# FutureSDR/FutureSDR

Hardware: AMD Instinct MI355X
Metric: MSample/s through 127-tap C32 FIR→decim4→1k-FFT flowgraph @1/2/4/8 GPU (higher is better)
Workload: dtype f32; 1 GPU; fir127_decim4_fft1024; taps1=127, taps2=127, decim=4, fft_len=1024, parallelism=1 independent channels

## Files before the change

### futuresdr_amd/csrc/futuresdr_hip.hip

```cpp
#include <hip/hip_runtime.h>

#include <atomic>
#include <condition_variable>
#include <cstdio>
#include <cstring>
#include <cstdlib>
#include <deque>
#include <mutex>
#include <vector>
#include <algorithm>
#include <cmath>

#include "../../include/futuresdr_hip.h"


static thread_local char g_err[512];
static thread_local const char* g_err_ptr = "";

static void set_err(const char* msg) {
    snprintf(g_err, sizeof(g_err), "%s", msg);
    g_err_ptr = g_err;
}

extern "C" const char* fsdr_last_error(void) { return g_err_ptr; }
// ... 1667 lines not shown
    return ((((unsigned)(DFIRT_TILE + tpd + 12)) + 31u) & ~31u) + 8u;
}

template <int TPD>
__global__ __launch_bounds__(DFIRT_BLOCK) void k_fir_decim4_tpl(
    const float2* __restrict__ in, float2* __restrict__ out,
    const float* __restrict__ rtv ,
    long long n_out, long long n_in_valid) {
    static_assert(TPD % 4 == 0, "TPD must be a multiple of 4");
    const unsigned SP = dfirt_sp(TPD);
    extern __shared__ __attribute__((aligned(16))) char smem[];
    float* planes = (float*)smem;
    float* s_rt = planes + 4u * SP;

    const int tid = threadIdx.x;
    const unsigned span = 3 + 4 * (DFIRT_TILE + TPD + 8);
    for (long long tile = blockIdx.x;
         tile * (long long)DFIRT_TILE < n_out; tile += gridDim.x) {
        const long long out_base = tile * DFIRT_TILE;
        const long long in_base = out_base * 4;
        const unsigned eb = (unsigned)tid * DFIRT_R;
        float2 a01r = make_float2(0.f, 0.f), a23r = a01r;
        float2 a01i = a01r, a23i = a01r;
#pragma unroll
        for (int half = 0; half < 2; half++) {
            for (unsigned idx = tid; 2 * idx + 3 < span;
                 idx += DFIRT_BLOCK) {
                unsigned i = idx >> 1, vloc = idx & 1u;
                unsigned rel = 3 + 4 * i + 2 * half + vloc;
                if (rel >= span) continue;
                long long g = in_base + rel;
                float2 x = (g < n_in_valid) ? in[g] : make_float2(0.f, 0.f);
                planes[vloc * SP + i] = x.x;
                planes[(2 + vloc) * SP + i] = x.y;
            }
            if (half == 0)
                for (int i = tid; i < 4 * (TPD + 4); i += DFIRT_BLOCK)
                    s_rt[i] = rtv[i];
            __syncthreads();
#pragma unroll
            for (int vloc = 0; vloc < 2; vloc++) {
                const float* pre = planes + (unsigned)vloc * SP;
                const float* pim = planes + (unsigned)(2 + vloc) * SP;
                const float* rt =
                    s_rt + (unsigned)(2 * half + vloc) * (TPD + 4);
                float4 r0 = *(const float4*)&pre[eb];
                float4 r1 = *(const float4*)&pre[eb + 4];
                float4 i0 = *(const float4*)&pim[eb];
                float4 i1 = *(const float4*)&pim[eb + 4];
                float4 hc = *(const float4*)&rt[0];
                constexpr int NG = TPD / 4;
#pragma unroll 4
                for (int m = 0; m < NG; m++) {
                    const float4 rn = *(const float4*)&pre[eb + 4 * m + 8];
                    const float4 in_ = *(const float4*)&pim[eb + 4 * m + 8];
                    const float4 h4 = *(const float4*)&rt[4 * m + 4];
                    const float wr[8] = {r0.x, r0.y, r0.z, r0.w,
                                         r1.x, r1.y, r1.z, r1.w};
                    const float wi[8] = {i0.x, i0.y, i0.z, i0.w,
                                         i1.x, i1.y, i1.z, i1.w};
                    const float ht[4] = {hc.x, hc.y, hc.z, hc.w};
#pragma unroll
                    for (int tl = 0; tl < 4; tl++) {
                        const float h = ht[tl];
                        a01r.x = fmaf(wr[tl], h, a01r.x);
                        a01r.y = fmaf(wr[tl + 1], h, a01r.y);
                        a23r.x = fmaf(wr[tl + 2], h, a23r.x);
                        a23r.y = fmaf(wr[tl + 3], h, a23r.y);
                        a01i.x = fmaf(wi[tl], h, a01i.x);
                        a01i.y = fmaf(wi[tl + 1], h, a01i.y);
                        a23i.x = fmaf(wi[tl + 2], h, a23i.x);
                        a23i.y = fmaf(wi[tl + 3], h, a23i.y);
                    }
                    r0 = r1; r1 = rn;
                    i0 = i1; i1 = in_;
                    hc = h4;
                }
            }
            __syncthreads();
        }
        const float ar[4] = {a01r.x, a01r.y, a23r.x, a23r.y};
        const float ai[4] = {a01i.x, a01i.y, a23i.x, a23i.y};
#pragma unroll
        for (int j = 0; j < DFIRT_R; j++) {
            long long o = out_base + eb + j;
            if (o < n_out) out[o] = make_float2(ar[j], ai[j]);
        }
    }
}

typedef void (*dfir_tpl_fn)(const float2*, float2*, const float*, long long,
                            long long);

__global__ void k_fir_decim_generic_cf32(const float2* __restrict__ in,
                                         float2* __restrict__ out,
                                         const float* __restrict__ taps,
                                         int n_taps, long long decim,
                                         long long n_out,
                                         long long n_in_valid) {
    long long stride = (long long)gridDim.x * blockDim.x;
    for (long long k = blockIdx.x * (long long)blockDim.x + threadIdx.x;
         k < n_out; k += stride) {
        float sre = 0.f, sim = 0.f;
        long long base = decim - 1 + k * decim;
        for (int t = 0; t < n_taps; t++) {
            float2 x = (base + t < n_in_valid) ? in[base + t]
                                               : make_float2(0.f, 0.f);
            float h = taps[n_taps - 1 - t];
            sre = fmaf(x.x, h, sre);
            sim = fmaf(x.y, h, sim);
        }
        out[k] = make_float2(sre, sim);
    }
}

__global__ __launch_bounds__(256) void k_fir_ccf32(
    const float2* __restrict__ in, float2* __restrict__ out,
    const float2* __restrict__ taps, int n_taps, long long n_out,
    long long n_in_valid) {
    const unsigned TILE = 1024;
    const unsigned elems = TILE + n_taps - 1;
    extern __shared__ __attribute__((aligned(16))) char smem[];
    float2* s_x = (float2*)smem;
    float2* s_h = s_x + elems;
    const int tid = threadIdx.x;
    for (long long tile = blockIdx.x; tile * (long long)TILE < n_out;
         tile += gridDim.x) {
        const long long out_base = tile * TILE;
        for (unsigned i = tid; i < elems; i += 256) {
            long long g = out_base + i;
            s_x[i] = (g < n_in_valid) ? in[g] : make_float2(0.f, 0.f);
        }
        for (int i = tid; i < n_taps; i += 256)
            s_h[i] = taps[n_taps - 1 - i];
        __syncthreads();
        for (int j = 0; j < 4; j++) {
            unsigned k = tid + j * 256;
            float sre = 0.f, sim = 0.f;
            for (int t = 0; t < n_taps; t++) {
                float2 x = s_x[k + t];
                float2 h = s_h[t];
                sre = fmaf(x.x, h.x, sre);
                sre = fmaf(-x.y, h.y, sre);
                sim = fmaf(x.x, h.y, sim);
                sim = fmaf(x.y, h.x, sim);
            }
            long long o = out_base + k;
            if (o < n_out) out[o] = make_float2(sre, sim);
        }
        __syncthreads();
    }
}

__global__ void k_moving_avg_chunks(const float* __restrict__ in,
                                    float* __restrict__ partial, int width,
                                    long long frames, int n_chunks,
                                    int chunk_frames, float decay) {
    if ((width & 3) == 0) {
        int w4 = width >> 2;
        long long id = blockIdx.x * (long long)blockDim.x + threadIdx.x;
        long long total = (long long)n_chunks * w4;
        long long stride = (long long)gridDim.x * blockDim.x;
        for (; id < total; id += stride) {
            int c = (int)(id / w4);
            int b4 = (int)(id - (long long)c * w4);
            long long f0 = (long long)c * chunk_frames;
            long long f1 = f0 + chunk_frames;
            if (f1 > frames) f1 = frames;
            float4 p = make_float4(0.f, 0.f, 0.f, 0.f);
            const float om = 1.0f - decay;
            for (long long f = f0; f < f1; f++) {
                float4 t = *(const float4*)&in[f * width + 4 * b4];
                p.x = isfinite(t.x) ? om * p.x + decay * t.x : om * p.x;
                p.y = isfinite(t.y) ? om * p.y + decay * t.y : om * p.y;
                p.z = isfinite(t.z) ? om * p.z + decay * t.z : om * p.z;
                p.w = isfinite(t.w) ? om * p.w + decay * t.w : om * p.w;
            }
            *(float4*)&partial[(long long)c * width + 4 * b4] = p;
        }
        return;
    }
    long long id = blockIdx.x * (long long)blockDim.x + threadIdx.x;
    long long total = (long long)n_chunks * width;
    long long stride = (long long)gridDim.x * blockDim.x;
    for (; id < total; id += stride) {
        int c = (int)(id / width);
        int b = (int)(id - (long long)c * width);
        long long f0 = (long long)c * chunk_frames;
        long long f1 = f0 + chunk_frames;
        if (f1 > frames) f1 = frames;
        float p = 0.f;
        for (long long f = f0; f < f1; f++) {
            float t = in[f * width + b];
            if (isfinite(t))
                p = (1.0f - decay) * p + decay * t;
            else
                p *= 1.0f - decay;
        }
        partial[(long long)c * width + b] = p;
    }
}

__global__ void k_moving_avg_combine(const float* __restrict__ partial,
                                     float* __restrict__ avg,
                                     float* __restrict__ out ,
                                     int width, long long frames,
                                     int n_chunks, int chunk_frames,
                                     float decay) {
    __shared__ float red[256];
    const int b = blockIdx.x;
    if (b >= width) return;
    const float om = 1.0f - decay;
    float acc = 0.f;
    for (int c = threadIdx.x; c < n_chunks; c += blockDim.x) {
        long long end = (long long)(c + 1) * chunk_frames;
        if (end > frames) end = frames;
        acc += powf(om, (float)(frames - end)) *
               partial[(long long)c * width + b];
    }
    red[threadIdx.x] = acc;
    __syncthreads();
    for (int s = 128; s > 0; s >>= 1) {
        if (threadIdx.x < s) red[threadIdx.x] += red[threadIdx.x + s];
        __syncthreads();
    }
    if (threadIdx.x == 0) {
        float a = powf(om, (float)frames) * avg[b] + red[0];
        avg[b] = a;
        if (out) out[b] = a;
    }
}

__global__ __launch_bounds__(256) void k_xlating_decim_ccf32(
    const float2* __restrict__ in, float2* __restrict__ out,
    const float2* __restrict__ taps , int n_taps,
    long long decim, long long n_out, long long n_in_valid, double theta,
    float p0r, float p0i) {
    extern __shared__ __attribute__((aligned(16))) char smem[];
    float2* s_h = (float2*)smem;
    for (int i = threadIdx.x; i < n_taps; i += blockDim.x) s_h[i] = taps[i];
    __syncthreads();
    long long stride = (long long)gridDim.x * blockDim.x;
    for (long long k = blockIdx.x * (long long)blockDim.x + threadIdx.x;
         k < n_out; k += stride) {
        float sre = 0.f, sim = 0.f;
        long long base = decim - 1 + k * decim;
        for (int t = 0; t < n_taps; t++) {
            float2 x = (base + t < n_in_valid) ? in[base + t]
                                               : make_float2(0.f, 0.f);
            float2 hh = s_h[t];
            sre = fmaf(x.x, hh.x, sre);
            sre = fmaf(-x.y, hh.y, sre);
            sim = fmaf(x.x, hh.y, sim);
            sim = fmaf(x.y, hh.x, sim);
        }
        double a = theta * (double)(k + 1);
        a -= 6.283185307179586 * floor(a * 0.15915494309189535);
        float s, cth;
        __sincosf((float)a, &s, &cth);
        float pr = cth * p0r - s * p0i;
        float pi = cth * p0i + s * p0r;
        out[k] = make_float2(sre * pr - sim * pi, sre * pi + sim * pr);
    }
}

#define XT_BLOCK 256
#define XT_R 2
#define XT_TILE (XT_BLOCK * XT_R)

__global__ __launch_bounds__(XT_BLOCK) void k_xlating_decim_tiled_ccf32(
    const float2* __restrict__ in, float2* __restrict__ out,
    const float2* __restrict__ taps , int n_taps,
    int decim, long long n_out, long long n_in_valid, double theta,
    float p0r, float p0i, int span) {
    extern __shared__ __attribute__((aligned(16))) char smem[];
    float* s_re = (float*)smem;
    float* s_im = s_re + plane_floats((unsigned)span);
    float* s_hr = s_im + plane_floats((unsigned)span);
    float* s_hi = s_hr + n_taps;
    for (int i = threadIdx.x; i < n_taps; i += XT_BLOCK) {
        s_hr[i] = taps[i].x;
        s_hi[i] = taps[i].y;
    }
    const long long tiles = (n_out + XT_TILE - 1) / XT_TILE;
    for (long long tile = blockIdx.x; tile < tiles; tile += gridDim.x) {
        const long long out_base = tile * XT_TILE;
        const long long in_base = decim - 1 + out_base * decim;
        __syncthreads();
        for (int i = threadIdx.x; i < span; i += XT_BLOCK) {
            long long g = in_base + i;
            float2 v = (g < n_in_valid) ? in[g] : make_float2(0.f, 0.f);
            s_re[lds_pad((unsigned)i)] = v.x;
            s_im[lds_pad((unsigned)i)] = v.y;
        }
        __syncthreads();
#pragma unroll
        for (int r = 0; r < XT_R; r++) {
            long long k = out_base + threadIdx.x + r * XT_BLOCK;
            if (k >= n_out) break;
            unsigned rel = (unsigned)((k - out_base) * decim);
            float sre = 0.f, sim = 0.f;
#pragma unroll 4
            for (int t = 0; t < n_taps; t++) {
                unsigned a = lds_pad(rel + (unsigned)t);
                float xr = s_re[a], xi = s_im[a];
                float hr = s_hr[t], hi = s_hi[t];
                sre = fmaf(xr, hr, sre);
                sre = fmaf(-xi, hi, sre);
                sim = fmaf(xr, hi, sim);
                sim = fmaf(xi, hr, sim);
            }
            double a = theta * (double)(k + 1);
            a -= 6.283185307179586 * floor(a * 0.15915494309189535);
            float s, cth;
            __sincosf((float)a, &s, &cth);
            float pr = cth * p0r - s * p0i;
            float pi = cth * p0i + s * p0r;
            out[k] = make_float2(sre * pr - sim * pi, sre * pi + sim * pr);
        }
    }
}

__global__ void k_cmul_conj(const float2* __restrict__ a,
                            const float2* __restrict__ b,
                            float2* __restrict__ o, long long n) {
    long long stride = (long long)gridDim.x * blockDim.x;
    for (long long i = blockIdx.x * (long long)blockDim.x + threadIdx.x;
         i < n; i += stride) {
        float2 x = a[i], y = b[i];
        o[i] = make_float2(x.x * y.x + x.y * y.y, x.y * y.x - x.x * y.y);
    }
}

__global__ void k_divide_mag(const float2* __restrict__ a,
                             const float* __restrict__ b,
                             float* __restrict__ o, long long n) {
    long long stride = (long long)gridDim.x * blockDim.x;
    for (long long i = blockIdx.x * (long long)blockDim.x + threadIdx.x;
         i < n; i += stride) {
        float2 x = a[i];
        o[i] = sqrtf(x.x * x.x + x.y * x.y) / b[i];
    }
}

__global__ void k_moving_sum(const float* __restrict__ in,
                             float* __restrict__ out, int width, int len,
                             long long n_out_items) {
    long long stride = (long long)gridDim.x * blockDim.x;
    long long total = n_out_items * width;
    for (long long id = blockIdx.x * (long long)blockDim.x + threadIdx.x;
         id < total; id += stride) {
        long long i = id / width;
        int q = (int)(id - i * width);
        float sum = 0.f;
        for (int t = 0; t < len; t++) sum += in[(i + t) * width + q];
        out[id] = sum;
    }
}

__global__ void k_pfb_dots(const float2* __restrict__ in,
                           float2* __restrict__ fb,
                           const float* __restrict__ part ,
                           int N, int tpf, int D, long long steps,
                           long long p_before, long long bufbase) {
    long long id = blockIdx.x * (long long)blockDim.x + threadIdx.x;
    long long total = steps * N;
    long long stride = (long long)gridDim.x * blockDim.x;
// ... 848 lines not shown

extern "C" fsdr_filter* fsdr_mag2_create(void) {
    fsdr_filter* f = create_common(K_MAG2);
    if (!f) return nullptr;
    f->item_out = 4;
    return f;
}

extern "C" fsdr_filter* fsdr_xlating_fir_cf32_create(const float* taps,
                                                     size_t n_taps,
                                                     size_t decimation,
                                                     float offset,
                                                     float sample_rate) {
    if (!taps || n_taps == 0 || decimation < 2) {
        set_err("xlating fir: taps required, decimation must be >= 2");
        return nullptr;
    }
    fsdr_filter* f = create_common(K_XLATING);
    if (!f) return nullptr;
    f->n_taps = n_taps;
    f->decim = decimation;
    std::vector<float2> bpf(n_taps);
    for (size_t i = 0; i < n_taps; i++) {
        float ang = (float)i * 6.2831853071795864769f * offset / sample_rate;
        float2 rot = make_float2(cosf(ang), sinf(ang));
        size_t src_i = i;
        bpf[n_taps - 1 - src_i] =
            make_float2(rot.x * taps[src_i], rot.y * taps[src_i]);
    }
    if (hipMalloc(&f->d_taps, bpf.size() * sizeof(float2)) != hipSuccess ||
        hipMemcpy(f->d_taps, bpf.data(), bpf.size() * sizeof(float2),
                  hipMemcpyHostToDevice) != hipSuccess) {
        set_err("bpf taps upload failed");
        delete f;
        return nullptr;
    }
    f->theta = -6.2831853071795864769f * offset * (float)decimation /
               sample_rate;
    f->rot_re = 1.0f;
    f->rot_im = 0.0f;
    f->n_taps_padded = (int)n_taps;
    return f;
}

extern "C" fsdr_filter* fsdr_pfb_channelizer_create(size_t num_channels,
                                                    const float* taps,
                                                    size_t n_taps,
                                                    float oversample_rate) {
    if (num_channels <= 2 || !taps || n_taps < num_channels) {
        set_err("pfb: num_channels > 2 and taps.len() >= num_channels");
        return nullptr;
    }
    if (!(oversample_rate > 0.f) ||
        fmodf((float)num_channels, oversample_rate) != 0.f) {
        set_err("pfb: oversample rate must be N/i for i in [1, N]");
        return nullptr;
    }
    if ((num_channels & (num_channels - 1)) != 0 || num_channels < 4 ||
        num_channels > 4096) {
        set_err("pfb: num_channels must be a power of two in [4,4096] "
                "(FFT kernel constraint)");
        return nullptr;
    }
    fsdr_filter* f = create_common(K_PFB);
    if (!f) return nullptr;
    f->width = num_channels;
    f->decim = (size_t)((float)num_channels / oversample_rate);
    size_t tpf = (n_taps + num_channels - 1) / num_channels;
    f->history = tpf;
    f->n_taps = n_taps;
    std::vector<float> part(num_channels * tpf, 0.f);
    for (size_t i = 0; i < num_channels; i++) {
        size_t cnt = 0;
        for (size_t t = i; t < n_taps; t += num_channels)
            part[i * tpf + cnt++] = taps[t];
    }
    if (hipMalloc(&f->d_taps, part.size() * sizeof(float)) != hipSuccess ||
        hipMemcpy(f->d_taps, part.data(), part.size() * sizeof(float),
                  hipMemcpyHostToDevice) != hipSuccess) {
        set_err("pfb taps upload failed");
        delete f;
        return nullptr;
    }
    f->sub = fsdr_fft_cf32_create(num_channels, 1, 0, nullptr);
    if (!f->sub) {
        delete f;
        return nullptr;
    }
    return f;
}

extern "C" fsdr_filter* fsdr_moving_avg_create(size_t width,
                                               float decay_factor,
                                               size_t history) {
    if (width == 0 || history == 0 || !(decay_factor >= 0.f) ||
        decay_factor > 1.f) {
        set_err("decay_factor must be in [0,1], width/history > 0");
        return nullptr;
    }
    fsdr_filter* f = create_common(K_MOVAVG);
    if (!f) return nullptr;
    f->width = width;
    f->history = history;
    f->decay = decay_factor;
    f->item_in = f->item_out = 4;
    f->n_taps = width;
    if (hipMalloc(&f->d_avg, width * sizeof(float)) != hipSuccess ||
        hipMemset(f->d_avg, 0, width * sizeof(float)) != hipSuccess) {
        set_err("avg state alloc failed");
        delete f;
        return nullptr;
    }
    return f;
}

extern "C" size_t fsdr_filter_length(const fsdr_filter* f) {
    return f ? (f->kind == K_MAG2 ? 1 : f->n_taps) : 0;
}

extern "C" size_t fsdr_filter_item_sizes(const fsdr_filter* f,
                                         size_t* out_bytes) {
    if (!f) { if (out_bytes) *out_bytes = 8; return 8; }
    if (out_bytes) *out_bytes = f->item_out;
    return f->item_in;
}

extern "C" void fsdr_filter_destroy(fsdr_filter* f) {
    if (!f) return;
    if (f->sub) fsdr_filter_destroy(f->sub);
    if (f->d_avg) (void)hipFree(f->d_avg);
    if (f->d_taps) (void)hipFree(f->d_taps);
    if (f->d_rtaps) (void)hipFree(f->d_rtaps);
    if (f->d_mtaps) (void)hipFree(f->d_mtaps);
    if (f->d_mtaps32) (void)hipFree(f->d_mtaps32);
    if (f->d_twid) (void)hipFree(f->d_twid);
    if (f->d_chirp) (void)hipFree(f->d_chirp);
    if (f->d_B) (void)hipFree(f->d_B);
    if (f->d_in) (void)hipFree(f->d_in);
    if (f->d_out) (void)hipFree(f->d_out);
    if (f->d_scratch) (void)hipFree(f->d_scratch);
    if (f->d_hist) (void)hipFree(f->d_hist);
    delete f;
}


static int grid_for(long long work_items, int block) {
    long long g = (work_items + block - 1) / block;
    const long long cap = 256 * 32;
    if (g > cap) g = cap;
    if (g < 1) g = 1;
    return (int)g;
}

static int launch_fir_cf32(fsdr_filter* f, const void* d_in, void* d_out,
                           size_t n_out, size_t n_in, hipStream_t st) {
    if (n_out == 0) return FSDR_OK;
    long long tiles = ((long long)n_out + FIR_TILE_OUT - 1) / FIR_TILE_OUT;
    long long cap = 256 * 16;
    if (const char* e = getenv("FSDR_FIR_GRID_CAP")) cap = atoll(e);
    int grid = (int)std::min<long long>(tiles, cap);
    const char* mf32 = getenv("FSDR_FIR_MFMA32");
    if (f->kk_mfma && mf32 && atoi(mf32) != 0) {
        long long tiles32 =
            ((long long)n_out + MFIR32_TILE - 1) / MFIR32_TILE;
        long long cap32 = 256 * 64;
        if (const char* e = getenv("FSDR_FIR_GRID_CAP")) cap32 = atoll(e);
        int grid32 = (int)std::min<long long>(tiles32, cap32);
        unsigned elems32 = MFIR32_TILE + f->kk_mfma32 + 8;
        size_t lds32 = (2 * (size_t)((elems32 + 31u) & ~31u) +
                        f->kk_mfma32 + 36) * sizeof(float);
#define MFIR32_TPL_CASE(KV)                                                      case KV:                                                                         hipLaunchKernelGGL(HIP_KERNEL_NAME(k_fir_mfma32_tpl<KV>),                                       dim3(grid32), dim3(MFIR32_BLOCK), lds32, st,                                 (const float2*)d_in, (float2*)d_out,                                         f->d_mtaps32, (long long)n_out, (long long)n_in);         break;
        switch (f->kk_mfma32) {
            MFIR32_TPL_CASE(48)
            MFIR32_TPL_CASE(96)
            MFIR32_TPL_CASE(160)
            MFIR32_TPL_CASE(288)
            MFIR32_TPL_CASE(544)
            default:
                set_err("bad mfma32 K");
                return FSDR_ERR_INVALID;
        }
#undef MFIR32_TPL_CASE
        HIP_TRY(hipGetLastError());
        return FSDR_OK;
    }
    const char* mf = getenv("FSDR_FIR_MFMA");
    if (f->kk_mfma && (!mf || atoi(mf) != 0)) {
        unsigned elems = MFIR_TILE + f->kk_mfma + 8;
        size_t lds = (2 * (size_t)((elems + 31u) & ~31u) + f->kk_mfma + 20)
                     * sizeof(float);
#define MFIR_TPL_CASE(KV)                                                        case KV:                                                                         hipLaunchKernelGGL(HIP_KERNEL_NAME(k_fir_mfma_tpl<KV>), dim3(grid),                             dim3(MFIR_BLOCK), lds, st, (const float2*)d_in,                              (float2*)d_out, f->d_mtaps, (long long)n_out,                                (long long)n_in);                                         break;
        switch (f->kk_mfma) {
            MFIR_TPL_CASE(32)
            MFIR_TPL_CASE(64)
            MFIR_TPL_CASE(96)
            MFIR_TPL_CASE(144)
            MFIR_TPL_CASE(272)
            MFIR_TPL_CASE(528)
            default:
                set_err("bad mfma K");
                return FSDR_ERR_INVALID;
        }
#undef MFIR_TPL_CASE
        HIP_TRY(hipGetLastError());
        return FSDR_OK;
    }
    if (f->tp_tpl) {
        unsigned elems = FIR_TILE_OUT + f->tp_tpl + 8;
        size_t lds = (2 * (size_t)((elems + 7u) & ~7u) + f->tp_tpl + 3) *
                     sizeof(float);
#define FIR_TPL_CASE(TPV)                                                        case TPV:                                                                        hipLaunchKernelGGL(HIP_KERNEL_NAME(k_fir_cf32_tpl<TPV>),                                        dim3(grid), dim3(FIR_BLOCK), lds, st,                                        (const float2*)d_in, (float2*)d_out, f->d_rtaps,                             (long long)n_out, (long long)n_in);                       break;
        switch (f->tp_tpl) {
            FIR_TPL_CASE(17)
            FIR_TPL_CASE(33)
            FIR_TPL_CASE(65)
            FIR_TPL_CASE(129)
            FIR_TPL_CASE(257)
            FIR_TPL_CASE(513)
            default:
                set_err("bad template tap count");
                return FSDR_ERR_INVALID;
        }
#undef FIR_TPL_CASE
        HIP_TRY(hipGetLastError());
        return FSDR_OK;
    }
    unsigned elems = FIR_TILE_OUT + f->n_taps_padded - 1 + 6;
    size_t lds = (2 * (size_t)plane_floats(elems) + f->n_taps_padded + 4) *
                 sizeof(float);
    hipLaunchKernelGGL(k_fir_cf32, dim3(grid), dim3(FIR_BLOCK), lds, st,
                       (const float2*)d_in, (float2*)d_out, f->d_taps,
                       f->n_taps_padded, (long long)n_out, (long long)n_in);
    HIP_TRY(hipGetLastError());
    return FSDR_OK;
}

static int launch_decim_cf32(fsdr_filter* f, const void* d_in, void* d_out,
                             size_t n_out, size_t n_in, hipStream_t st) {
    if (n_out == 0) return FSDR_OK;
    const char* dmf = getenv("FSDR_DECIM_MFMA");
    if (f->decim == 4 && f->kk_mfma && (!dmf || atoi(dmf) != 0)) {
        long long tiles = ((long long)n_out + MDFIR_TILE - 1) / MDFIR_TILE;
        long long cap = 256 * 64;
        if (const char* e = getenv("FSDR_FIR_GRID_CAP")) cap = atoll(e);
        int grid = (int)std::min<long long>(tiles, cap);
        unsigned elemsP = MDFIR_TILE + f->kk_mfma + 8;
        size_t lds = (4 * (size_t)((elemsP + 31u) & ~31u) +
                      4 * ((size_t)f->kk_mfma + 16)) * sizeof(float);
#define MDFIR_TPL_CASE(KV)                                                       case KV:                                                                         hipLaunchKernelGGL(HIP_KERNEL_NAME(k_decim4_mfma_tpl<KV>),                                      dim3(grid), dim3(MDFIR_BLOCK), lds, st,                                      (const float2*)d_in, (float2*)d_out, f->d_mtaps,                             (long long)n_out, (long long)n_in);                       break;
        switch (f->kk_mfma) {
            MDFIR_TPL_CASE(20)
            MDFIR_TPL_CASE(32)
            MDFIR_TPL_CASE(48)
            MDFIR_TPL_CASE(80)
            MDFIR_TPL_CASE(144)
            default:
                set_err("bad decim mfma K");
                return FSDR_ERR_INVALID;
        }
#undef MDFIR_TPL_CASE
        HIP_TRY(hipGetLastError());
        return FSDR_OK;
    }
    if (f->decim == 4 && f->tp_tpl) {
        long long tiles = ((long long)n_out + DFIRT_TILE - 1) / DFIRT_TILE;
        long long cap = 256 * 64;
        if (const char* e = getenv("FSDR_FIR_GRID_CAP")) cap = atoll(e);
        int grid = (int)std::min<long long>(tiles, cap);
        size_t lds = (4 * (size_t)dfirt_sp(f->tp_tpl) +
                      4 * ((size_t)f->tp_tpl + 4)) * sizeof(float);
#define DFIR_TPL_CASE(TPV)                                                       case TPV:                                                                        hipLaunchKernelGGL(HIP_KERNEL_NAME(k_fir_decim4_tpl<TPV>),                                      dim3(grid), dim3(DFIRT_BLOCK), lds, st,                                      (const float2*)d_in, (float2*)d_out, f->d_rtaps,                             (long long)n_out, (long long)n_in);                       break;
        switch (f->tp_tpl) {
            DFIR_TPL_CASE(8)
            DFIR_TPL_CASE(16)
            DFIR_TPL_CASE(32)
            DFIR_TPL_CASE(64)
            DFIR_TPL_CASE(128)
            default:
                set_err("bad decim template tap count");
                return FSDR_ERR_INVALID;
        }
#undef DFIR_TPL_CASE
        HIP_TRY(hipGetLastError());
        return FSDR_OK;
    }
    if (f->decim == 4) {
        unsigned elems = DFIR_TILE_OUT * 4 + f->n_taps_padded - 1 + 20;
        size_t lds = (2 * (size_t)plane_floats(elems) + f->n_taps_padded + 4)
                     * sizeof(float);
        long long tiles =
            ((long long)n_out + DFIR_TILE_OUT - 1) / DFIR_TILE_OUT;
        int grid = (int)std::min<long long>(tiles, 256 * 8);
        hipLaunchKernelGGL(k_fir_decim4_cf32, dim3(grid), dim3(DFIR_BLOCK),
                           lds, st, (const float2*)d_in, (float2*)d_out,
                           f->d_taps, f->n_taps_padded, (long long)n_out,
                           (long long)n_in);
    } else {
        hipLaunchKernelGGL(k_fir_decim_generic_cf32,
                           dim3(grid_for((long long)n_out, 256)), dim3(256),
                           0, st, (const float2*)d_in, (float2*)d_out,
                           f->d_taps,
                           f->n_taps_padded,
                           (long long)f->decim, (long long)n_out,
                           (long long)n_in);
    }
    HIP_TRY(hipGetLastError());
// ... 66 lines not shown
extern "C" int fsdr_fft_bulk_dev(fsdr_filter* f, const void* d_in,
                                 void* d_out, void* d_mag, size_t frames,
                                 void* stream) {
    REQUIRE_GPU();
    if (!f || f->kind != K_FFT_CF32) {
        set_err("fft_bulk: not an fft filter");
        return FSDR_ERR_INVALID;
    }
    return launch_fft(f, d_in, d_out, frames, (hipStream_t)stream,
                      (float*)d_mag);
}

extern "C" int fsdr_filter_dev(fsdr_filter* f, const void* d_in, size_t n_in,
                               void* d_out, size_t n_out, void* stream,
                               fsdr_filter_result* r) {
    REQUIRE_GPU();
    if (!f || !r) { set_err("null argument"); return FSDR_ERR_INVALID; }
    hipStream_t st = (hipStream_t)stream;
    switch (f->kind) {
        case K_FIR_CF32: {
            *r = fir_status(n_in, f->n_taps, n_out);
            return launch_fir_cf32(f, d_in, d_out, r->produced, n_in, st);
        }
        case K_FIR_F32: {
            *r = fir_status(n_in, f->n_taps, n_out);
            if (r->produced == 0) return FSDR_OK;
            unsigned elems = 1024 + f->n_taps_padded - 1;
            size_t lds = (size_t)elems * sizeof(float);
            long long tiles = ((long long)r->produced + 1023) / 1024;
            int grid = (int)std::min<long long>(tiles, 256 * 16);
            hipLaunchKernelGGL(k_fir_f32, dim3(grid), dim3(256), lds, st,
                               (const float*)d_in, (float*)d_out, f->d_taps,
                               f->n_taps_padded, (long long)r->produced,
                               (long long)n_in);
            HIP_TRY(hipGetLastError());
            return FSDR_OK;
        }
        case K_DECIM_CF32: {
            *r = decim_status(f->decim, n_in, f->n_taps, n_out);
            return launch_decim_cf32(f, d_in, d_out, r->produced, n_in, st);
        }
        case K_RESAMP_CF32: {
            *r = resamp_status(f->interp, f->decim, f->n_taps, n_in, n_out);
            if (r->produced == 0) return FSDR_OK;
            const char* dmf = getenv("FSDR_DECIM_MFMA");
            if (f->sub && f->sub->kk_mfma && (!dmf || atoi(dmf) != 0)) {
                return launch_decim_cf32(f->sub,
                                         (const float2*)d_in - 3, d_out,
                                         r->produced, n_in + 3, st);
            }
            size_t tpp = f->n_taps / f->interp;
            long long span = (long long)(RS_TILE - 1) * f->decim /
                                 f->interp + tpp + 2;
            size_t lds_t = (2 * (size_t)plane_floats((unsigned)span) +
                            f->n_taps) * sizeof(float);
            const char* rt = getenv("FSDR_RESAMP_TILED");
            if (lds_t <= 64 * 1024 && (!rt || atoi(rt) != 0)) {
                long long tiles =
                    ((long long)r->produced + RS_TILE - 1) / RS_TILE;
                int grid = (int)std::min<long long>(tiles, 256 * 64);
                hipLaunchKernelGGL(k_resamp_tiled_cf32, dim3(grid),
                                   dim3(RS_BLOCK), lds_t, st,
                                   (const float2*)d_in, (float2*)d_out,
                                   f->d_taps, (int)f->n_taps,
                                   (int)f->interp, (int)f->decim,
                                   (long long)r->produced, (long long)n_in,
                                   (int)span);
                HIP_TRY(hipGetLastError());
                return FSDR_OK;
            }
            size_t lds = f->n_taps * sizeof(float);
            hipLaunchKernelGGL(k_resamp_cf32,
                               dim3(grid_for((long long)r->produced, 256)),
                               dim3(256), lds, st, (const float2*)d_in,
                               (float2*)d_out, f->d_taps, (int)f->n_taps,
                               (int)f->interp, (int)f->decim,
                               (long long)r->produced, (long long)n_in);
            HIP_TRY(hipGetLastError());
            return FSDR_OK;
        }
        case K_FFT_CF32: {
            size_t m = n_in < n_out ? n_in : n_out;
            m = (m / f->fft_len) * f->fft_len;
            size_t cap = f->fft_len * 32;
            if (m > cap) m = cap;
            r->consumed = r->produced = m;
            r->status = FSDR_BOTH_SUFFICIENT;
            return launch_fft(f, d_in, d_out, m / f->fft_len, st);
        }
        case K_FIR_CCF32: {
            *r = fir_status(n_in, f->n_taps, n_out);
            if (r->produced == 0) return FSDR_OK;
            unsigned elems = 1024 + f->n_taps - 1;
            size_t lds = ((size_t)elems + f->n_taps) * sizeof(float2);
            long long tiles = ((long long)r->produced + 1023) / 1024;
            int grid = (int)std::min<long long>(tiles, 256 * 64);
            hipLaunchKernelGGL(k_fir_ccf32, dim3(grid), dim3(256), lds, st,
                               (const float2*)d_in, (float2*)d_out,
                               (const float2*)f->d_taps, (int)f->n_taps,
                               (long long)r->produced, (long long)n_in);
            HIP_TRY(hipGetLastError());
            return FSDR_OK;
        }
        case K_XLATING: {
            *r = decim_status(f->decim, n_in, f->n_taps, n_out);
            if (r->produced == 0) return FSDR_OK;
            long long span = (long long)(XT_TILE - 1) * f->decim +
                             f->n_taps + 2;
            size_t lds_t = (2 * (size_t)plane_floats((unsigned)span) +
                            2 * f->n_taps) * sizeof(float);
            const char* xt = getenv("FSDR_XLATING_TILED");
            if (lds_t <= 64 * 1024 && (!xt || atoi(xt) != 0)) {
                long long tiles =
                    ((long long)r->produced + XT_TILE - 1) / XT_TILE;
                int grid = (int)std::min<long long>(tiles, 256 * 64);
                hipLaunchKernelGGL(k_xlating_decim_tiled_ccf32,
                                   dim3(grid), dim3(XT_BLOCK), lds_t, st,
                                   (const float2*)d_in, (float2*)d_out,
                                   (const float2*)f->d_taps,
                                   (int)f->n_taps, (int)f->decim,
                                   (long long)r->produced, (long long)n_in,
                                   (double)f->theta, f->rot_re, f->rot_im,
                                   (int)span);
                HIP_TRY(hipGetLastError());
            } else {
                size_t lds = f->n_taps * sizeof(float2);
                hipLaunchKernelGGL(
                    k_xlating_decim_ccf32,
                    dim3(grid_for((long long)r->produced, 256)), dim3(256),
                    lds, st, (const float2*)d_in, (float2*)d_out,
                    (const float2*)f->d_taps, (int)f->n_taps,
                    (long long)f->decim, (long long)r->produced,
                    (long long)n_in, f->theta, f->rot_re, f->rot_im);
                HIP_TRY(hipGetLastError());
            }
            {
                double a = (double)f->theta * (double)r->produced;
                double cs = cos(a), sn = sin(a);
                float nr = (float)(cs * f->rot_re - sn * f->rot_im);
                float ni = (float)(cs * f->rot_im + sn * f->rot_re);
                f->rot_re = nr;
                f->rot_im = ni;
            }
            return FSDR_OK;
        }
        case K_PFB:
            set_err("pfb channelizer uses fsdr_pfb_channelizer_run_dev "
                    "(multi-output block)");
            return FSDR_ERR_INVALID;
        case K_MOVAVG: {
            size_t in_frames = n_in / f->width;
            size_t out_frames = n_out / f->width;
            size_t cons = 0, prod = 0, i = f->i_state;
            while (cons < in_frames && prod < out_frames) {
                if (++i == f->history) { i = 0; prod++; }
                cons++;
            }
            r->consumed = cons * f->width;
            r->produced = prod * f->width;
            r->status = FSDR_BOTH_SUFFICIENT;
            if (cons == 0) return FSDR_OK;
            if (prod <= 1 &&
                (prod == 0 || f->i_state + cons == f->history)) {
                int cf = 64;
                int nch = (int)((cons + cf - 1) / cf);
                if (nch > 1024) { nch = 1024; cf = (int)((cons + nch - 1) / nch); }
                int rc = ensure_dev(&f->d_scratch, &f->d_scratch_bytes,
                                    (size_t)nch * f->width * 4);
                if (rc) return rc;
                hipLaunchKernelGGL(
                    k_moving_avg_chunks,
                    dim3(grid_for((long long)nch * f->width, 256)),
                    dim3(256), 0, st, (const float*)d_in,
                    (float*)f->d_scratch, (int)f->width, (long long)cons,
                    nch, cf, f->decay);
                HIP_TRY(hipGetLastError());
                hipLaunchKernelGGL(k_moving_avg_combine,
                                   dim3((unsigned)f->width), dim3(256), 0,
                                   st, (const float*)f->d_scratch, f->d_avg,
                                   prod ? (float*)d_out : nullptr,
                                   (int)f->width, (long long)cons, nch, cf,
                                   f->decay);
                HIP_TRY(hipGetLastError());
                f->i_state = i;
                return FSDR_OK;
            }
            hipLaunchKernelGGL(k_moving_avg,
                               dim3((unsigned)((f->width + 255) / 256)),
                               dim3(256), 0, st, (const float*)d_in,
                               (float*)d_out, f->d_avg, (int)f->width,
                               (long long)cons, (int)f->i_state,
                               (int)f->history, f->decay);
            HIP_TRY(hipGetLastError());
            f->i_state = i;
            return FSDR_OK;
        }
        case K_MAG2: {
            size_t m = n_in < n_out ? n_in : n_out;
            r->consumed = r->produced = m;
            r->status = FSDR_BOTH_SUFFICIENT;
            if (m == 0) return FSDR_OK;
            hipLaunchKernelGGL(k_mag2, dim3(grid_for((long long)m, 256)),
                               dim3(256), 0, st, (const float2*)d_in,
                               (float*)d_out, (long long)m);
            HIP_TRY(hipGetLastError());
            return FSDR_OK;
        }
    }
    set_err("unknown filter kind");
    return FSDR_ERR_INVALID;
}

extern "C" int fsdr_filter_host(fsdr_filter* f, const void* in, size_t n_in,
                                void* out, size_t n_out,
                                fsdr_filter_result* r) {
    REQUIRE_GPU();
    if (!f || !r) { set_err("null argument"); return FSDR_ERR_INVALID; }
    int rc = ensure_dev(&f->d_in, &f->d_in_bytes, n_in * f->item_in + 64);
    if (rc) return rc;
    rc = ensure_dev(&f->d_out, &f->d_out_bytes, n_out * f->item_out + 64);
    if (rc) return rc;
    if (n_in)
        HIP_TRY(hipMemcpy(f->d_in, in, n_in * f->item_in,
                          hipMemcpyHostToDevice));
    rc = fsdr_filter_dev(f, f->d_in, n_in, f->d_out, n_out, nullptr, r);
    if (rc) return rc;
    HIP_TRY(hipStreamSynchronize(nullptr));
    if (r->produced)
        HIP_TRY(hipMemcpy(out, f->d_out, r->produced * f->item_out,
                          hipMemcpyDeviceToHost));
    return FSDR_OK;
}

extern "C" int fsdr_pfb_channelizer_run_dev(fsdr_filter* f,
                                            const void* d_in, size_t n_in,
                                            void* d_out,
                                            size_t out_cap_per_chan,
                                            void* stream,
                                            size_t* produced_per_chan) {
    REQUIRE_GPU();
    if (!f || f->kind != K_PFB) {
        set_err("not a pfb channelizer");
        return FSDR_ERR_INVALID;
    }
    hipStream_t st = (hipStream_t)stream;
    size_t N = f->width, tpf = f->history, D = f->decim;
    size_t prefill = N * tpf;
    size_t steps = n_in > prefill ? (n_in - prefill) / D : 0;
    if (steps > out_cap_per_chan) steps = out_cap_per_chan;
    if (produced_per_chan) *produced_per_chan = steps;
    if (steps == 0) return FSDR_OK;
    int rc = ensure_dev(&f->d_in, &f->d_in_bytes, steps * N * 8);
    if (rc) return rc;
    int rc2 = ensure_dev(&f->d_out, &f->d_out_bytes, steps * N * 8);
    if (rc2) return rc2;
    hipLaunchKernelGGL(k_pfb_dots,
                       dim3(grid_for((long long)(steps * N), 256)),
                       dim3(256), 0, st, (const float2*)d_in,
                       (float2*)f->d_in, (const float*)f->d_taps, (int)N,
                       (int)tpf, (int)D, (long long)steps,
                       (long long)prefill, (long long)0);
    HIP_TRY(hipGetLastError());
    rc = launch_fft(f->sub, f->d_in, f->d_out, steps, st);
    if (rc) return rc;
    hipLaunchKernelGGL(k_pfb_scatter,
                       dim3(grid_for((long long)(steps * N), 256)),
                       dim3(256), 0, st, (const float2*)f->d_out,
                       (float2*)d_out, (int)N, (long long)steps,
                       (long long)out_cap_per_chan);
    HIP_TRY(hipGetLastError());
    return FSDR_OK;
}

extern "C" int fsdr_pfb_channelizer_stream_dev(
    fsdr_filter* f, const void* d_chunk, size_t n, void* d_out,
    size_t out_cap_per_chan, void* stream, size_t* produced_per_chan,
    size_t* consumed) {
    REQUIRE_GPU();
    if (!f || f->kind != K_PFB) {
        set_err("not a pfb channelizer");
        return FSDR_ERR_INVALID;
    }
    hipStream_t st = (hipStream_t)stream;
    size_t N = f->width, tpf = f->history, D = f->decim;
    size_t prefill = N * tpf, W = N * tpf;
    size_t p = f->pfb_pushes;
    size_t T = p < W ? p : W;
    size_t fill = p < prefill ? std::min(prefill - p, n) : 0;
    size_t steps = (p + n >= prefill) ? (p + n - prefill) / D -
                                            (p > prefill ? (p - prefill) / D
                                                         : 0)
                                      : 0;
    if (steps > out_cap_per_chan) steps = out_cap_per_chan;
    size_t cons = fill + steps * D;
    if (cons > n) cons = n;
    if (produced_per_chan) *produced_per_chan = steps;
    if (consumed) *consumed = cons;
    if (cons == 0) return FSDR_OK;
    int rc = ensure_dev(&f->d_scratch, &f->d_scratch_bytes,
                        (T + cons) * 8);
    if (rc) return rc;
    if (T)
        HIP_TRY(hipMemcpyAsync(f->d_scratch, f->d_hist, T * 8,
                               hipMemcpyDeviceToDevice, st));
    HIP_TRY(hipMemcpyAsync((char*)f->d_scratch + T * 8, d_chunk, cons * 8,
                           hipMemcpyDeviceToDevice, st));
    if (steps) {
        rc = ensure_dev(&f->d_in, &f->d_in_bytes, steps * N * 8);
        if (rc) return rc;
        rc = ensure_dev(&f->d_out, &f->d_out_bytes, steps * N * 8);
        if (rc) return rc;
        hipLaunchKernelGGL(k_pfb_dots,
                           dim3(grid_for((long long)(steps * N), 256)),
                           dim3(256), 0, st, (const float2*)f->d_scratch,
                           (float2*)f->d_in, (const float*)f->d_taps,
                           (int)N, (int)tpf, (int)D, (long long)steps,
                           (long long)(p + fill), (long long)(p - T));
        HIP_TRY(hipGetLastError());
        rc = launch_fft(f->sub, f->d_in, f->d_out, steps, st);
        if (rc) return rc;
        hipLaunchKernelGGL(k_pfb_scatter,
                           dim3(grid_for((long long)(steps * N), 256)),
                           dim3(256), 0, st, (const float2*)f->d_out,
                           (float2*)d_out, (int)N, (long long)steps,
                           (long long)out_cap_per_chan);
        HIP_TRY(hipGetLastError());
    }
    size_t newT = std::min(W, T + cons);
    rc = ensure_dev(&f->d_hist, &f->d_hist_bytes, W * 8);
    if (rc) return rc;
    HIP_TRY(hipMemcpyAsync(f->d_hist,
                           (char*)f->d_scratch + (T + cons - newT) * 8,
                           newT * 8, hipMemcpyDeviceToDevice, st));
    f->pfb_pushes = p + cons;
    return FSDR_OK;
// ... 965 lines not shown
```

### include/futuresdr_hip.h

```cpp
#ifndef FUTURESDR_HIP_H
#define FUTURESDR_HIP_H

#include <stddef.h>
#include <stdint.h>

#ifdef __cplusplus
extern "C" {
#endif

typedef struct { float re, im; } fsdr_cf32;

typedef enum {
    FSDR_INSUFFICIENT_INPUT  = 0,
    FSDR_INSUFFICIENT_OUTPUT = 1,
    FSDR_BOTH_SUFFICIENT     = 2,
} fsdr_status;

typedef struct {
    size_t      consumed;
    size_t      produced;
    fsdr_status status;
} fsdr_filter_result;

enum {
    FSDR_OK              = 0,
    FSDR_ERR_NO_GPU      = 1,
    FSDR_ERR_HIP         = 2,
    FSDR_ERR_INVALID     = 3,
    FSDR_ERR_UNSUPPORTED = 4,
};

int         fsdr_device_count(void);
int         fsdr_set_device(int device);
int         fsdr_synchronize(void);
const char* fsdr_last_error(void);
const char* fsdr_version(void);

typedef struct fsdr_filter fsdr_filter;

fsdr_filter* fsdr_fir_cf32_create(const float* taps, size_t n_taps);
fsdr_filter* fsdr_fir_f32_create(const float* taps, size_t n_taps);
fsdr_filter* fsdr_fir_ccf32_create(const fsdr_cf32* taps, size_t n_taps);
fsdr_filter* fsdr_decim_fir_cf32_create(size_t decimation,
                                        const float* taps, size_t n_taps);
fsdr_filter* fsdr_resamp_cf32_create(size_t interp, size_t decim,
                                     const float* taps, size_t n_taps);
fsdr_filter* fsdr_fft_cf32_create(size_t len, int inverse, int fft_shift,
                                  const float* normalize);
fsdr_filter* fsdr_mag2_create(void);
fsdr_filter* fsdr_xlating_fir_cf32_create(const float* taps, size_t n_taps,
                                          size_t decimation, float offset,
                                          float sample_rate);
fsdr_filter* fsdr_moving_avg_create(size_t width, float decay_factor,
                                    size_t history);

size_t fsdr_filter_length(const fsdr_filter* f);

int fsdr_filter_host(fsdr_filter* f, const void* in, size_t n_in,
                     void* out, size_t n_out, fsdr_filter_result* r);
int fsdr_filter_dev(fsdr_filter* f, const void* d_in, size_t n_in,
                    void* d_out, size_t n_out, void* stream,
                    fsdr_filter_result* r);
int fsdr_fft_bulk_dev(fsdr_filter* f, const void* d_in, void* d_out,
                      void* d_mag, size_t frames, void* stream);
void fsdr_filter_destroy(fsdr_filter* f);

int fsdr_cmul_dev(const void* d_a, size_t n_a, const void* d_b, size_t n_b,
                  void* d_out, size_t n_out, void* stream, size_t* m);
int fsdr_cmul_host(const void* a, size_t n_a, const void* b, size_t n_b,
                   void* out, size_t n_out, size_t* m);

int fsdr_rotator_dev(const void* d_in, void* d_out, size_t n,
                     float phase_incr_angle, float phase0_re,
                     float phase0_im, void* stream, float* final_re,
                     float* final_im);

fsdr_filter* fsdr_pfb_channelizer_create(size_t num_channels,
                                         const float* taps, size_t n_taps,
                                         float oversample_rate);
int fsdr_pfb_channelizer_run_dev(fsdr_filter* f, const void* d_in,
                                 size_t n_in, void* d_out,
                                 size_t out_cap_per_chan, void* stream,
                                 size_t* produced_per_chan);
int fsdr_pfb_channelizer_stream_dev(fsdr_filter* f, const void* d_chunk,
                                    size_t n, void* d_out,
                                    size_t out_cap_per_chan, void* stream,
                                    size_t* produced_per_chan,
                                    size_t* consumed);

int fsdr_cmul_conj_dev(const void* d_a, size_t n_a, const void* d_b,
                       size_t n_b, void* d_out, size_t n_out, void* stream,
                       size_t* m);
int fsdr_divide_mag_dev(const void* d_a, size_t n_a, const void* d_b,
                        size_t n_b, void* d_out, size_t n_out, void* stream,
                        size_t* m);
int fsdr_wlan_moving_sum_dev(const void* d_in, size_t n_in, void* d_out,
                             size_t n_out, size_t len, int is_complex,
                             void* stream, size_t* produced);

typedef struct fsdr_wlan_rx fsdr_wlan_rx;
fsdr_wlan_rx* fsdr_wlan_rx_create(void);
void fsdr_wlan_rx_destroy(fsdr_wlan_rx* rx);
size_t fsdr_wlan_sync_short_run(fsdr_wlan_rx* rx, const fsdr_cf32* sig,
                                const fsdr_cf32* abs48, const float* cor,
                                size_t n, fsdr_cf32* out, size_t out_cap,
                                size_t* tag_idx, float* tag_freq,
                                size_t tag_cap, size_t* n_tags,
                                size_t* consumed_out);
size_t fsdr_wlan_sync_long_run(fsdr_wlan_rx* rx, const fsdr_cf32* in,
                               size_t n, const size_t* tag_idx,
                               const float* tag_freq, size_t num_tags,
                               fsdr_cf32* out, size_t out_cap,
                               size_t* frame_off, float* frame_freq,
                               size_t frame_cap, size_t* num_frames);

int fsdr_mfma_ubench(int grid, int iters, double* tflops, void* stream);
int fsdr_chain_ubench(int mode, double* tflops, void* stream);

int fsdr_dev_alloc(void** d_ptr, size_t bytes);
int fsdr_dev_free(void* d_ptr);
int fsdr_memcpy_h2d(void* d_dst, const void* src, size_t bytes);
int fsdr_memcpy_d2h(void* dst, const void* d_src, size_t bytes);
int fsdr_fill_uniform_cf32(void* d_ptr, size_t n, uint64_t seed,
                           uint64_t offset, void* stream);

double fsdr_kaiser_beta(double max_ripple);
void   fsdr_kaiser_window(size_t len, double beta, double* out);
size_t fsdr_firdes_kaiser_lowpass_f32(double cutoff, double transition_bw,
                                      double max_ripple, float* out,
                                      size_t cap);
int fsdr_firdes_lowpass_kaiser_n_f32(size_t n_taps, double beta,
                                     double cutoff, float* out);

typedef struct fsdr_chain fsdr_chain;
fsdr_chain* fsdr_chain_create(const float* taps1, size_t n_taps1,
                              const float* taps2, size_t n_taps2,
                              size_t decim, size_t fft_len);
int fsdr_chain_run_dev(fsdr_chain* c, const void* d_in, size_t n_in,
                       void* d_out, size_t out_cap,
                       void* d_mag, size_t mag_cap,
                       void* stream, size_t* consumed, size_t* produced);
void fsdr_chain_destroy(fsdr_chain* c);

typedef struct fsdr_ring fsdr_ring;
fsdr_ring* fsdr_ring_create(size_t n_buffers, size_t items_per_buffer,
                            size_t item_bytes, size_t reserved_items);
int  fsdr_ring_writer_acquire(fsdr_ring* r, void** host_ptr, size_t* items);
int  fsdr_ring_writer_commit(fsdr_ring* r, size_t items);
int  fsdr_ring_reader_acquire(fsdr_ring* r, void** dev_ptr, size_t* items);
int  fsdr_ring_reader_release_consumed(fsdr_ring* r, size_t consumed,
                                       void* stream);
int  fsdr_ring_reader_release(fsdr_ring* r);
void fsdr_ring_destroy(fsdr_ring* r);

typedef struct fsdr_ring_d2h fsdr_ring_d2h;
fsdr_ring_d2h* fsdr_ring_d2h_create(size_t n_buffers,
                                    size_t items_per_buffer,
                                    size_t item_bytes);
int  fsdr_ring_d2h_writer_acquire(fsdr_ring_d2h* r, void** dev_ptr,
                                  size_t* items, void* stream);
int  fsdr_ring_d2h_writer_commit(fsdr_ring_d2h* r, size_t items,
                                 void* stream);
int  fsdr_ring_d2h_reader_acquire(fsdr_ring_d2h* r, void** host_ptr,
                                  size_t* items);
int  fsdr_ring_d2h_reader_release(fsdr_ring_d2h* r);
void fsdr_ring_d2h_destroy(fsdr_ring_d2h* r);

typedef struct fsdr_fg fsdr_fg;
fsdr_fg* fsdr_fg_create(void);
int  fsdr_fg_add_null_source_cf32(fsdr_fg* fg);
int  fsdr_fg_add_vector_source_cf32(fsdr_fg* fg, const fsdr_cf32* data,
                                    size_t n);
int  fsdr_fg_add_head(fsdr_fg* fg, unsigned long long n);
int  fsdr_fg_add_filter(fsdr_fg* fg, fsdr_filter* f);
int  fsdr_fg_add_null_sink(fsdr_fg* fg);
int  fsdr_fg_add_vector_sink(fsdr_fg* fg);
int  fsdr_fg_stream(fsdr_fg* fg, int src_block, int dst_block);
int  fsdr_fg_run(fsdr_fg* fg);
unsigned long long fsdr_fg_n_received(fsdr_fg* fg, int block);
size_t fsdr_fg_vector_sink_get(fsdr_fg* fg, int block, void* out,
                               size_t cap_bytes);
void fsdr_fg_destroy(fsdr_fg* fg);
size_t fsdr_filter_item_sizes(const fsdr_filter* f, size_t* out_bytes);

#ifdef __cplusplus
}
#endif
#endif
```

Measured before the change: 182,900 MSample/s.

## Skip negligible moving-average history chunks and batch loads in chunk kernel

Adds a decay horizon so that input frames whose weight falls below float precision are skipped: chunk kernels and the combine step start at chunk c0. The frame/output counting loop is replaced with closed-form arithmetic, and the per-chunk loop loads 16 frames at once to expose memory-level parallelism. This targets the moving-average block, which is not part of the FIR→decim→FFT chain being measured, so the benchmark should be largely unaffected. The skip relies on underflow-level truncation and slightly changes numerics, with an env var to disable it.

Result: faster. 187,400 MSample/s, median of 6 (+2.4%).

```diff
diff --git a/futuresdr_amd/csrc/futuresdr_hip.hip b/futuresdr_amd/csrc/futuresdr_hip.hip
--- a/futuresdr_amd/csrc/futuresdr_hip.hip
+++ b/futuresdr_amd/csrc/futuresdr_hip.hip
@@ -1843,51 +1843,96 @@
     }
 }
 
+#define MOVAVG_BATCH 16
+
+__device__ __forceinline__ float movavg_step_v4(float p, float t, float om,
+                                                float decay) {
+#pragma clang fp contract(off)
+    const float m = om * p;
+    return isfinite(t) ? fmaf(decay, t, m) : m;
+}
+
+__device__ __forceinline__ float movavg_step_s(float p, float t, float om,
+                                               float decay) {
+#pragma clang fp contract(off)
+    const float m = om * p;
+    const float d = decay * t;
+    return isfinite(t) ? m + d : m;
+}
+
 __global__ void k_moving_avg_chunks(const float* __restrict__ in,
                                     float* __restrict__ partial, int width,
                                     long long frames, int n_chunks,
-                                    int chunk_frames, float decay) {
+                                    int chunk_frames, float decay, int c0) {
+    const float om = 1.0f - decay;
     if ((width & 3) == 0) {
         int w4 = width >> 2;
         long long id = blockIdx.x * (long long)blockDim.x + threadIdx.x;
-        long long total = (long long)n_chunks * w4;
+        long long total = (long long)(n_chunks - c0) * w4;
         long long stride = (long long)gridDim.x * blockDim.x;
         for (; id < total; id += stride) {
-            int c = (int)(id / w4);
-            int b4 = (int)(id - (long long)c * w4);
+            int lc = (int)(id / w4);
+            int b4 = (int)(id - (long long)lc * w4);
+            int c = c0 + lc;
             long long f0 = (long long)c * chunk_frames;
             long long f1 = f0 + chunk_frames;
             if (f1 > frames) f1 = frames;
             float4 p = make_float4(0.f, 0.f, 0.f, 0.f);
-            const float om = 1.0f - decay;
-            for (long long f = f0; f < f1; f++) {
+            long long f = f0;
+            for (; f + MOVAVG_BATCH <= f1; f += MOVAVG_BATCH) {
+                v4f t[MOVAVG_BATCH];
+#pragma unroll
+                for (int u = 0; u < MOVAVG_BATCH; u++)
+                    t[u] = *(const v4f*)&in[(f + u) * width + 4 * b4];
+                static_assert(MOVAVG_BATCH == 16, "operand list below");
+                asm volatile(""
+                             : "+v"(t[0]), "+v"(t[1]), "+v"(t[2]), "+v"(t[3]),
+                               "+v"(t[4]), "+v"(t[5]), "+v"(t[6]), "+v"(t[7]),
+                               "+v"(t[8]), "+v"(t[9]), "+v"(t[10]),
+                               "+v"(t[11]), "+v"(t[12]), "+v"(t[13]),
+                               "+v"(t[14]), "+v"(t[15]));
+#pragma unroll
+                for (int u = 0; u < MOVAVG_BATCH; u++) {
+                    p.x = movavg_step_v4(p.x, t[u].x, om, decay);
+                    p.y = movavg_step_v4(p.y, t[u].y, om, decay);
+                    p.z = movavg_step_v4(p.z, t[u].z, om, decay);
+                    p.w = movavg_step_v4(p.w, t[u].w, om, decay);
+                }
+            }
+            for (; f < f1; f++) {
                 float4 t = *(const float4*)&in[f * width + 4 * b4];
-                p.x = isfinite(t.x) ? om * p.x + decay * t.x : om * p.x;
-                p.y = isfinite(t.y) ? om * p.y + decay * t.y : om * p.y;
-                p.z = isfinite(t.z) ? om * p.z + decay * t.z : om * p.z;
-                p.w = isfinite(t.w) ? om * p.w + decay * t.w : om * p.w;
+                p.x = movavg_step_v4(p.x, t.x, om, decay);
+                p.y = movavg_step_v4(p.y, t.y, om, decay);
+                p.z = movavg_step_v4(p.z, t.z, om, decay);
+                p.w = movavg_step_v4(p.w, t.w, om, decay);
             }
             *(float4*)&partial[(long long)c * width + 4 * b4] = p;
         }
         return;
     }
     long long id = blockIdx.x * (long long)blockDim.x + threadIdx.x;
-    long long total = (long long)n_chunks * width;
+    long long total = (long long)(n_chunks - c0) * width;
     long long stride = (long long)gridDim.x * blockDim.x;
     for (; id < total; id += stride) {
-        int c = (int)(id / width);
-        int b = (int)(id - (long long)c * width);
+        int lc = (int)(id / width);
+        int b = (int)(id - (long long)lc * width);
+        int c = c0 + lc;
         long long f0 = (long long)c * chunk_frames;
         long long f1 = f0 + chunk_frames;
         if (f1 > frames) f1 = frames;
         float p = 0.f;
-        for (long long f = f0; f < f1; f++) {
-            float t = in[f * width + b];
-            if (isfinite(t))
-                p = (1.0f - decay) * p + decay * t;
-            else
-                p *= 1.0f - decay;
-        }
+        long long f = f0;
+        for (; f + MOVAVG_BATCH <= f1; f += MOVAVG_BATCH) {
+            float t[MOVAVG_BATCH];
+#pragma unroll
+            for (int u = 0; u < MOVAVG_BATCH; u++)
+                t[u] = in[(f + u) * width + b];
+#pragma unroll
+            for (int u = 0; u < MOVAVG_BATCH; u++)
+                p = movavg_step_s(p, t[u], om, decay);
+        }
+        for (; f < f1; f++)
+            p = movavg_step_s(p, in[f * width + b], om, decay);
         partial[(long long)c * width + b] = p;
     }
 }
@@ -1897,13 +1942,14 @@
                                      float* __restrict__ out ,
                                      int width, long long frames,
                                      int n_chunks, int chunk_frames,
-                                     float decay) {
+                                     float decay, int c0) {
     __shared__ float red[256];
     const int b = blockIdx.x;
     if (b >= width) return;
     const float om = 1.0f - decay;
     float acc = 0.f;
     for (int c = threadIdx.x; c < n_chunks; c += blockDim.x) {
+        if (c < c0) continue;
         long long end = (long long)(c + 1) * chunk_frames;
         if (end > frames) end = frames;
         acc += powf(om, (float)(frames - end)) *
@@ -3058,6 +3104,63 @@
     return (int)g;
 }
 
+static long long movavg_horizon(float decay) {
+    const double om = fabs((double)(1.0f - decay));
+    if (om == 0.0) return 1;
+    if (!(om < 1.0)) return 0;
+    const double h = ceil(160.0 * M_LN2 / -log(om));
+    if (!(h < 9.0e18)) return 0;
+    return h < 1.0 ? 1 : (long long)h;
+}
+
+static void movavg_count(size_t in_frames, size_t out_frames, size_t history,
+                         size_t* cons, size_t* prod, size_t* i) {
+    *cons = *prod = 0;
+    if (out_frames == 0 || in_frames == 0) return;
+    const size_t first = history - *i;
+    size_t need = SIZE_MAX;
+    if (out_frames - 1 <= (SIZE_MAX - first) / history)
+        need = first + (out_frames - 1) * history;
+    const size_t c = in_frames < need ? in_frames : need;
+    *cons = c;
+    if (c < first) {
+        *i += c;
+    } else {
+        *prod = 1 + (c - first) / history;
+        *i = (c - first) % history;
+    }
+}
+
+static int movavg_plan(size_t frames, float decay, bool skip, int* cf_out,
+                       int* nch_out) {
+    int cf = 64;
+    int nch = (int)((frames + cf - 1) / cf);
+    if (nch > 1024) { nch = 1024; cf = (int)((frames + nch - 1) / nch); }
+    *cf_out = cf;
+    *nch_out = nch;
+    int c0 = 0;
+    const long long H = movavg_horizon(decay);
+    if (skip && H > 0 && (long long)frames > H) {
+        c0 = (int)(((long long)frames - H) / cf);
+        if (c0 > nch - 1) c0 = nch - 1;
+    }
+    return c0;
+}
+
+extern "C" void fsdr_moving_avg_count(size_t in_frames, size_t out_frames,
+                                      size_t history, size_t* i_state,
+                                      size_t* consumed, size_t* produced) {
+    movavg_count(in_frames, out_frames, history, consumed, produced,
+                 i_state);
+}
+
+extern "C" int fsdr_moving_avg_plan(size_t frames, float decay_factor,
+                                    int skip, int* chunk_frames,
+                                    int* n_chunks) {
+    return movavg_plan(frames, decay_factor, skip != 0, chunk_frames,
+                       n_chunks);
+}
+
 static int launch_fir_cf32(fsdr_filter* f, const void* d_in, void* d_out,
                            size_t n_out, size_t n_in, hipStream_t st) {
     if (n_out == 0) return FSDR_OK;
@@ -3430,35 +3533,36 @@
             size_t in_frames = n_in / f->width;
             size_t out_frames = n_out / f->width;
             size_t cons = 0, prod = 0, i = f->i_state;
-            while (cons < in_frames && prod < out_frames) {
-                if (++i == f->history) { i = 0; prod++; }
-                cons++;
-            }
+            movavg_count(in_frames, out_frames, f->history, &cons, &prod,
+                         &i);
             r->consumed = cons * f->width;
             r->produced = prod * f->width;
             r->status = FSDR_BOTH_SUFFICIENT;
             if (cons == 0) return FSDR_OK;
             if (prod <= 1 &&
                 (prod == 0 || f->i_state + cons == f->history)) {
-                int cf = 64;
-                int nch = (int)((cons + cf - 1) / cf);
-                if (nch > 1024) { nch = 1024; cf = (int)((cons + nch - 1) / nch); }
+                const char* sk = getenv("FSDR_MOVAVG_SKIP");
+                int cf, nch;
+                const int c0 = movavg_plan(cons, f->decay,
+                                           !sk || atoi(sk) != 0, &cf, &nch);
                 int rc = ensure_dev(&f->d_scratch, &f->d_scratch_bytes,
                                     (size_t)nch * f->width * 4);
                 if (rc) return rc;
+                const long long live =
+                    (long long)(nch - c0) *
+                    ((f->width & 3) == 0 ? f->width / 4 : f->width);
                 hipLaunchKernelGGL(
-                    k_moving_avg_chunks,
-                    dim3(grid_for((long long)nch * f->width, 256)),
+                    k_moving_avg_chunks, dim3(grid_for(live, 256)),
                     dim3(256), 0, st, (const float*)d_in,
                     (float*)f->d_scratch, (int)f->width, (long long)cons,
-                    nch, cf, f->decay);
+                    nch, cf, f->decay, c0);
                 HIP_TRY(hipGetLastError());
                 hipLaunchKernelGGL(k_moving_avg_combine,
                                    dim3((unsigned)f->width), dim3(256), 0,
                                    st, (const float*)f->d_scratch, f->d_avg,
                                    prod ? (float*)d_out : nullptr,
                                    (int)f->width, (long long)cons, nch, cf,
-                                   f->decay);
+                                   f->decay, c0);
                 HIP_TRY(hipGetLastError());
                 f->i_state = i;
                 return FSDR_OK;
diff --git a/include/futuresdr_hip.h b/include/futuresdr_hip.h
--- a/include/futuresdr_hip.h
+++ b/include/futuresdr_hip.h
@@ -53,6 +53,11 @@
                                           float sample_rate);
 fsdr_filter* fsdr_moving_avg_create(size_t width, float decay_factor,
                                     size_t history);
+void fsdr_moving_avg_count(size_t in_frames, size_t out_frames,
+                           size_t history, size_t* i_state,
+                           size_t* consumed, size_t* produced);
+int fsdr_moving_avg_plan(size_t frames, float decay_factor, int skip,
+                         int* chunk_frames, int* n_chunks);
 
 size_t fsdr_filter_length(const fsdr_filter* f);
 
```
